# Gotbread/sdf-playground

Measured on AMD Instinct MI355X. Metric: Mrays/s (primary+secondary), labyrinth scene, 3840x2160, higher is better.
Workload: dtype f32

## Files before the change

sdf_playground_amd/buildlib.py:

```python
import hashlib
import os
import re
import subprocess
import sys
from concurrent.futures import ThreadPoolExecutor

HERE = os.path.dirname(os.path.abspath(__file__))
CSRC = os.path.join(HERE, "csrc")
LIB = os.path.join(HERE, "libsdfr.so")
OBJDIR = os.path.join(HERE, "build")
SOURCES = ["sdfr_api.cpp", "sdfr_comm.cpp", "sdfr_hlsl.cpp", "sdfr_jit.cpp", "sdfr_kernels.hip", "sdfr_post.hip"]
GROUP_SOURCE = "sdfr_kernels_group.hip"
ARCH = "gfx950"
_REV = ["-mllvm", "-greedy-reverse-local-assignment"]
_MAXMEM = ["-mllvm", "-amdgpu-sched-strategy=max-memory-clause"]
_TOPDOWN = ["-mllvm", "-misched-prera-direction=topdown"]
_MAXILP = ["-mllvm", "-amdgpu-sched-strategy=max-ilp"]
SCENE_FLAGS = {"SceneFractal": _MAXILP, "SceneCoordinateMaterial": _REV, "SceneTerrain": _REV, "SceneTiling": _REV,
               "SceneCubeSea": _MAXMEM, "SceneShell": _MAXMEM, "SceneLense": _TOPDOWN}


def scene_registry():
    text = open(os.path.join(CSRC, "sdfr_perpixel.h")).read()
    return [(int(i), n) for i, n in re.findall(r"X\((\d+), (Scene\w+)\)", text)]


def group_flags(g, override=None):
    groups = scene_groups()
    flags = []
    table = dict(SCENE_FLAGS)
    table.update(override or {})
    for i, name in scene_registry():
        if i % groups == g:
            flags += [f for f in table.get(name, []) if f not in flags or f == "-mllvm"]
    return flags


FLAGS = ["--offload-arch=" + ARCH, "-std=c++17", "-O3", "-ffp-contract=off", "-fno-slp-vectorize", "-fPIC", "-x", "hip", "-Wno-unused-result",
         "-Wno-unknown-pragmas", "-I" + CSRC]


def scene_groups():
    text = open(os.path.join(CSRC, "sdfr_perpixel.h")).read()
    return int(re.search(r"#define SDFR_GROUPS (\d+)", text).group(1))


def _deps():
    return [os.path.join(CSRC, f) for f in os.listdir(CSRC)] + [os.path.join(os.path.dirname(HERE), "include", "sdfr.h")]


def _stale():
    if not os.path.exists(LIB):
        return True
    t = os.path.getmtime(LIB)
    return any(os.path.getmtime(d) > t for d in _deps())


def build(force=False, verbose=False, extra=(), out=None, jobs=None, scene_flags=None):
    if out is None and not force and not _stale():
        return LIB
    hipcc = os.environ.get("HIPCC", "/opt/rocm/bin/hipcc")
    extra = list(extra)
    objdir = os.path.join(OBJDIR, hashlib.sha1(" ".join(extra).encode()).hexdigest()[:10] if extra else "default")
    os.makedirs(objdir, exist_ok=True)
    units = [(s, [], os.path.join(objdir, s + ".o")) for s in SOURCES]
    for g in range(scene_groups()):
        flags = group_flags(g, scene_flags)
        tag = "" if flags == group_flags(g) else "." + hashlib.sha1(" ".join(flags).encode()).hexdigest()[:8]
        units.append((GROUP_SOURCE, ["-DSDFR_GROUP=%d" % g] + flags, os.path.join(objdir, "%s.%d%s.o" % (GROUP_SOURCE, g, tag))))
    newest_dep = max(os.path.getmtime(d) for d in _deps())

    def compile_unit(u):
        src, defs, obj = u
        if not force and os.path.exists(obj) and os.path.getmtime(obj) > newest_dep:
            return
        cmd = [hipcc] + FLAGS + extra + defs + ["-c", os.path.join(CSRC, src), "-o", obj]
        if verbose:
            print(" ".join(cmd), file=sys.stderr)
        subprocess.run(cmd, check=True)

    with ThreadPoolExecutor(max_workers=jobs or min(8, os.cpu_count() or 1)) as pool:
        list(pool.map(compile_unit, sorted(units, key=lambda u: u[0] != GROUP_SOURCE)))
    cmd = [hipcc, "--offload-arch=" + ARCH, "-fPIC", "-shared"] + [u[2] for u in units] + ["-o", out or LIB]
    if verbose:
        print(" ".join(cmd), file=sys.stderr)
    subprocess.run(cmd, check=True)
    return out or LIB


if __name__ == "__main__":
    build(force="--force" in sys.argv, verbose="-v" in sys.argv)
    print(LIB)
```

sdf_playground_amd/csrc/sdfr_pixel.h:

```cpp
#pragma once
#include "sdfr_frame.h"
#include "sdfr_lib.h"

namespace sdfr {

struct PixelRay
{
	vec3 dir;
	vec3 right_ray, bottom_ray;
};
SDF_HD PixelRay pixel_ray(const FrameU &U, int px, int py)
{
	float sx = ((float)px + 0.5f) / U.widthf * 2.f - 1.f;
	float sy = 1.f - ((float)py + 0.5f) / U.heightf * 2.f;
	vec3 d = U.front + sx * U.right + sy * U.top;
	float invlen = rcp1(length(d));
	PixelRay r;
	r.dir = d * invlen;
	r.right_ray = U.ddx * U.right * invlen;
	r.bottom_ray = U.ddy * U.top * invlen;
	return r;
}
SDF_HD RayRec primary_ray(const FrameU &U, const PixelRay &pr)
{
// ... 11 lines not shown
	f.has_transparent = ray_has_transparent(r);
	f.is_shadow = ray_is_shadow(r);
	f.last_transparent_pos = f.has_transparent ? r.pos : V3s(0.f);
	return f;
}

SDF_HD int queue_next(uint64_t depths, int slots)
{
	int best = 0;
	uint32_t best_depth = (uint32_t)(depths & 0xffu);
	for (int i = 1; i < slots; ++i)
	{
		uint32_t d = (uint32_t)((depths >> (8 * i)) & 0xffu);
		if (d < best_depth) { best = i; best_depth = d; }
	}
	return best;
}
SDF_HD int queue_free(uint64_t depths, int slots)
{
	int i = 0;
	for (; i < slots; ++i)
		if (((depths >> (8 * i)) & 0xffu) == RAY_DEPTH_INVALID) break;
	return i;
}
SDF_HD uint64_t queue_set_depth(uint64_t depths, int slot, uint32_t d)
{
	return (depths & ~(0xffull << (8 * slot))) | ((uint64_t)d << (8 * slot));
}
#define SDFR_QUEUE_EMPTY 0xffffffffffffffffull

struct DebugFlags
{
	int plane_on;
	int show_on;
};
SDF_HD DebugFlags debug_flags(const FrameU &U)
{
	DebugFlags f;
	f.plane_on = U.debug_plane_on;
	f.show_on = U.show_on;
#if defined(__HIP_DEVICE_COMPILE__)
	asm volatile("" : "+v"(f.plane_on), "+v"(f.show_on));
#endif
	return f;
}
SDF_HD bool frame_needs_debug(const FrameU &U) { return U.debug_plane_on != 0 || U.show_on == 0; }

template <class Scene, bool DBG>
SDF_HD float map_geometry(const FrameU &U, const DebugFlags &F, const typename Scene::RayInv &R, vec3 p, vec3 dir, bool fast)
{
	if (!DBG)
		return Scene::dist(U, R, p, dir, fast);
	float d = 3e38f;
	if (F.show_on)
		d = Scene::dist(U, R, p, dir, fast);
	if (F.plane_on)
	{
		float plane = sd_plane_fast(p - V3(U.debug_x, U.debug_y, U.debug_z), dir, fast, U.debug_normal);
		return min1(d, plane);
	}
	return d;
}

struct GeoStep
{
	float camera_distance;
	vec3 right_off, bottom_off;
};
template <bool B>
struct VoidIf {};
template <>
struct VoidIf<true> { typedef void type; };
template <class Scene, class = void>
struct SceneReadsMarchState { static constexpr bool value = false; };
template <class Scene>
struct SceneReadsMarchState<Scene, typename VoidIf<Scene::geometry_reads_march_state>::type> { static constexpr bool value = true; };

template <class Scene, bool DBG>
SDF_HD float map_geometry_at(const FrameU &U, const DebugFlags &F, const typename Scene::RayInv &R, vec3 p, vec3 dir, bool fast, const GeoStep &gs)
{
	if (!DBG)
		return Scene::dist(U, R, p, dir, fast, gs);
	float d = 3e38f;
	if (F.show_on)
		d = Scene::dist(U, R, p, dir, fast, gs);
	if (F.plane_on)
	{
		float plane = sd_plane_fast(p - V3(U.debug_x, U.debug_y, U.debug_z), dir, fast, U.debug_normal);
		return min1(d, plane);
	}
	return d;
}

struct March
{
	vec3 start, dir;
	float t;
	float last_d;
	float last_safe;
	float factor;
	float d;
	uint32_t iter;
};
enum { MARCH_CONTINUE = 0, MARCH_HIT = 1, MARCH_MISS = 2 };

SDF_HD March march_begin(vec3 start, vec3 dir)
{
	March m;
	m.start = start;
	m.dir = dir;
	m.t = 0.f;
	m.last_d = 0.f;
	m.last_safe = 0.f;
	m.factor = 1.f;
	m.d = 0.f;
	m.iter = 0;
	return m;
}
SDF_HD vec3 march_pos(const March &m) { return mad(m.dir, m.t, m.start); }

SDF_HD int march_advance(March &m, float d, float dist_max, uint32_t iter_count, float dist_eps)
{
	m.d = d;
	const bool over = (m.factor > 1.f) & ((m.last_d + d) < m.last_d * m.factor);
	const bool out_of_range = m.t > dist_max;
	const bool stop = !over & (out_of_range | (d < dist_eps));
	const float t_fwd = m.t + d * m.factor;
	const float safe_fwd = m.t + d;
	m.last_d = over ? m.last_d : d;
	m.t = stop ? m.t : (over ? m.last_safe : t_fwd);
	m.last_safe = (over | stop) ? m.last_safe : safe_fwd;
	m.factor = over ? 1.f : m.factor;
	if (stop) return out_of_range ? MARCH_MISS : MARCH_HIT;
	m.iter++;
	return m.iter < iter_count ? MARCH_CONTINUE : MARCH_MISS;
}
SDF_HD void march_pre(March &m) { if (m.iter == 3) m.factor = 1.5f; }

SDF_HD vec3 grad_sample_pos(vec3 p, int axis, float eps)
{
	if (axis == 0) return p + V3(eps, 0.f, 0.f);
	if (axis == 1) return p + V3(0.f, eps, 0.f);
	return p + V3(0.f, 0.f, eps);
}

template <class...>
struct VoidOfN { typedef void type; };
template <class Scene, class = void>
struct SceneNormal
{
	static constexpr bool available = false;
	static SDF_HD void call(const FrameU &, const SurfacePoint &, NormalOut &) {}
};
template <class Scene>
struct SceneNormal<Scene, typename VoidOfN<decltype(&Scene::normal)>::type>
{
	static constexpr bool available = true;
	static SDF_HD void call(const FrameU &U, const SurfacePoint &sp, NormalOut &no) { Scene::normal(U, sp, no); }
};
template <class Scene>
SDF_HD NormalOut scene_normal(const FrameU &U, vec3 hit_pos, vec3 dir, float camera_distance, vec3 right_ray, vec3 bottom_ray)
{
	NormalOut no;
	no.sample_dist = U.grad_eps;
	no.normal = V3s(0.f);
	no.use_normal = false;
	if (SceneNormal<Scene>::available)
	{
		SurfacePoint sp;
		sp.pos = hit_pos;
		sp.dir = dir;
		sp.camera_distance = camera_distance;
		sp.right_off = right_ray;
		sp.bottom_off = bottom_ray;
		sp.normal = V3s(0.f);
		sp.iteration_count = 0u;
		sp.scene_distance = 0.f;
		SceneNormal<Scene>::call(U, sp, no);
	}
	return no;
}

template <class Scene, class = void>
struct SceneLights
{
	static constexpr bool available = false;
	static SDF_HD void call(const FrameU &, const SurfacePoint &, Light *, bool *, float &) {}
};
template <class Scene>
struct SceneLights<Scene, typename VoidOfN<decltype(&Scene::lights)>::type>
{
	static constexpr bool available = true;
	static SDF_HD void call(const FrameU &U, const SurfacePoint &sp, Light *L, bool *used, float &ambient) { Scene::lights(U, sp, L, used, ambient); }
};
template <class Scene, bool HasLights = SceneLights<Scene>::available>
struct SceneAmbient { static SDF_HD float get() { return Scene::ambient(); } };
template <class Scene>
struct SceneAmbient<Scene, true> { static SDF_HD float get() { return 0.075f; } };
template <class Scene, bool HasLights = SceneLights<Scene>::available>
struct SceneLightSlot { static SDF_HD bool get(const FrameU &U, int i, Light &L) { return Scene::light(U, i, L); } };
template <class Scene>
struct SceneLightSlot<Scene, true> { static SDF_HD bool get(const FrameU &, int, Light &) { return false; } };

struct HitInfo
{
	vec3 pos;
	float t;
	float d;
	uint32_t iter;
	vec3 normal;
	float sample_dist;
};

template <class Store>
struct Spawner
{
	Store &store;
	uint64_t depths;
	int count;
	int slots;
	SDF_HD Spawner(Store &s, uint64_t d, int c, int n) : store(s), depths(d), count(c), slots(n) {}
	SDF_HD void push(const RayRec &r)
	{
		if (count < slots)
		{
			int slot = queue_free(depths, slots);
			store.put(slot, r);
			depths = queue_set_depth(depths, slot, ray_depth(r));
			++count;
		}
	}
};

SDF_HD Material default_material(const FrameU &U, vec3 hit_pos)
{
	Material m;
	m.id = MAT_NONE;
	m.mpos = hit_pos;
	m.prop_x = 0.f;
	m.diffuse = V4(0.f, 0.f, 0.f, 1.f);
	m.specular = V4(0.f, 0.f, 0.f, 60.f);
	m.emissive = V3s(0.f);
	m.reflection = V3s(0.f);
	m.refraction = V3s(0.f);
	m.ior = 1.4f;
	m.normal = V4(0.f, 0.f, 0.f, 0.f);
	m.max_cost = U.max_cost_default;
	m.use_hdr = true;
	return m;
}

template <class Scene, bool DBG>
SDF_HD void map_material(const FrameU &U, const DebugFlags &F, const SurfacePoint &sp, Material &m)
{
	if (!DBG)
	{
		Scene::material(U, sp, m);
		return;
	}
	bool on_debug_plane = false;
	if (F.plane_on)
	{
		float plane = sd_plane(sp.pos - V3(U.debug_x, U.debug_y, U.debug_z), U.debug_normal);
		on_debug_plane = on_surface(U, plane);
	}
	if (on_debug_plane)
	{
		RayFlags nf;
		nf.has_transparent = false;
		nf.is_shadow = false;
		nf.last_transparent_pos = V3s(0.f);
		typename Scene::RayInv R0 = Scene::ray_setup(U, sp.dir, nf);
		float d;
		if constexpr (SceneReadsMarchState<Scene>::value)
		{
			GeoStep gs;
			gs.camera_distance = sp.camera_distance;
			gs.right_off = sp.right_off;
			gs.bottom_off = sp.bottom_off;
			d = Scene::dist(U, R0, sp.pos, sp.dir, false, gs);
		}
		else
			d = Scene::dist(U, R0, sp.pos, sp.dir, false);
		m.id = MAT_DISTANCE_PLANE;
		m.prop_x = d / U.debug_scale;
	}
	else
	{
		Scene::material(U, sp, m);
	}
}

template <class Scene, class = void>
struct RayEscapes
{
	static constexpr bool available = false;
	template <class R> static SDF_HD bool test(const FrameU &, const R &, vec3, vec3) { return false; }
};
template <class Scene>
struct RayEscapes<Scene, typename VoidOfN<decltype(&Scene::ray_escapes)>::type>
{
	static constexpr bool available = true;
	template <class R> static SDF_HD bool test(const FrameU &U, const R &r, vec3 p, vec3 dir) { return Scene::ray_escapes(U, r, p, dir); }
};

template <class Scene, class = void>
struct EscapesFrom
{
	static constexpr bool available = false;
	static SDF_HD float get(const FrameU &, vec3, vec3, float) { return 3e38f; }
};
template <class Scene>
struct EscapesFrom<Scene, typename VoidOfN<decltype(&Scene::escapes_from)>::type>
{
	static constexpr bool available = true;
	static SDF_HD float get(const FrameU &U, vec3 start, vec3 dir, float range) { return Scene::escapes_from(U, start, dir, range); }
};
template <class Scene, class = void>
struct InlineEscapedShadows { static constexpr bool value = false; };
template <class Scene>
struct InlineEscapedShadows<Scene, typename VoidOfN<decltype(Scene::inline_escaped_shadows)>::type>
{
	static constexpr bool value = Scene::inline_escaped_shadows && RayEscapes<Scene>::available;
};
struct InlineShadows
{
	vec3 acc;
	int budget;
	int taken;
};

template <class Scene, class Table, class Used>
SDF_HD bool light_in_slot(const FrameU &U, int i, const Table &table, const Used &table_used, Light &L)
{
	bool used = SceneLightSlot<Scene>::get(U, i, L);
	if (SceneLights<Scene>::available)
	{
		L = table[i];
		used = table_used[i];
	}
	if (i >= 1 && i <= U.extension_lights)
	{
		const float *E = U.ext_light[i - 1];
		L.pos = V3(E[0], E[1], E[2]);
		L.directional = false;
		L.extend = 0.25f;
		L.falloff = 0.25f;
		L.color = V3(E[3], E[4], E[5]);
		used = true;
	}
	return used;
}
SDF_HD vec3 light_colour(const Light &L)
{
	float falloff = 1.f;
	if (!L.directional) falloff = pow1(0.1f, L.falloff);
	return L.color * falloff;
}

template <class Scene, bool DBG, class Store, bool INL = false>
SDF_HD vec3 shade_hit(const FrameU &U, const DebugFlags &F, const RayRec &ray, const PixelRay &px, const HitInfo &hit, float max_range,
	float &hdr, Spawner<Store> &q, InlineShadows *inl = nullptr)
{
	bool added = false;
	const uint32_t depth = ray_depth(ray);
	const float inside_sign = ray_inside_sign(ray);
	const vec3 view_dir = ray.dir;

	SurfacePoint sp;
	sp.pos = hit.pos;
	sp.dir = ray.dir;
	sp.camera_distance = hit.t;
	sp.right_off = px.right_ray;
	sp.bottom_off = px.bottom_ray;
	sp.normal = hit.normal;
	sp.iteration_count = hit.iter;
	sp.scene_distance = hit.d;

	Material m = default_material(U, hit.pos);
	map_material<Scene, DBG>(U, F, sp, m);
	if (U.extension_marble_reflection != 0.f && (m.id == MAT_MARBLE_DARK || m.id == MAT_MARBLE_LIGHT)) m.reflection = V3s(U.extension_marble_reflection);

	vec3 out = V3s(0.f);
	if (!ray_is_shadow(ray))
	{
		float new_hdr = m.use_hdr ? 1.f : 0.f;
		hdr = lerp1(hdr, new_hdr, step1(hdr, 0.f));

		vec3 n = lerp(hit.normal, V3(m.normal.x, m.normal.y, m.normal.z), m.normal.w);

		if (any3(m.reflection) && inside_sign > 0.f && depth + 3 < m.max_cost)
		{
			vec3 rv = reflect(view_dir, n);
			RayRec c;
			c.pos = mad(rv, U.reflect_eps, hit.pos);
			c.dir = rv;
			c.contrib = m.reflection * ray.contrib;
			c.shadow_range = 0.f;
			c.bits = depth + 3;
			q.push(c);
		}
		if (any3(m.refraction) && depth + 4 < m.max_cost)
		{
			RayRec c;
			vec3 rv;
			if (inside_sign > 0.f)
			{
				rv = refract(view_dir, n, 1.f / m.ior);
				c.bits = (depth + 2) | RAY_INSIDE;
			}
			else
			{
				rv = refract(view_dir, -n, m.ior);
				c.bits = depth + 2;
			}
			c.pos = mad(rv, U.refract_eps, hit.pos);
			c.dir = rv;
			c.contrib = m.refraction * ray.contrib;
			c.shadow_range = 0.f;
			q.push(c);
		}

		vec3 diffuse = V3(m.diffuse.x, m.diffuse.y, m.diffuse.z);
		vec3 color = V3s(0.f);
		bool use_light = true;
		switch (m.id)
		{
		case MAT_ITER:
			color = color + mat_iter_heat(hit.iter, (uint32_t)(U.iter_count - 1));
			use_light = false;
			hdr = 0.f;
			break;
		case MAT_PLAIN:
			color = color + diffuse;
			use_light = false;
			break;
		case MAT_NORMAL1:
		{
			vec3 nc = max(n, 0.01f);
			nc = nc / max1(max1(nc.x, nc.y), nc.z);
			color = color + nc;
			use_light = false;
			hdr = 0.f;
			break;
		}
		case MAT_NORMAL2:
			color = color + abs(n);
			use_light = false;
			hdr = 0.f;
			break;
		case MAT_DISTANCE_PLANE:
			color = color + mat_debug_plane(m.prop_x);
			use_light = false;
			hdr = 0.f;
			break;
		case MAT_WOOD:
			diffuse = diffuse + mat_wood(m.mpos);
			break;
		case MAT_MARBLE_DARK:
			diffuse = diffuse + mat_marble(m.mpos, V3(0.556f, 0.478f, 0.541f));
			break;
		case MAT_MARBLE_LIGHT:
			diffuse = diffuse + mat_marble(m.mpos, V3(0.7f, 0.7f, 0.7f));
			break;
		case MAT_FIRE:
		{
			float fadeout = sat1(dot(-view_dir, n));
			vec4 fc = mat_fire(m.mpos, 1.f - fadeout);
			color = color + V3(fc.x, fc.y, fc.z);
			m.diffuse = V4(1.f, 1.f, 1.f, sat1(fc.w));
			break;
		}
		default:
			break;
		}

		if (m.diffuse.w < 1.f && depth + 2 < m.max_cost)
		{
			RayRec c;
			c.pos = hit.pos;
			c.dir = view_dir;
			c.contrib = (1.f - m.diffuse.w) * V3(m.diffuse.x, m.diffuse.y, m.diffuse.z) * ray.contrib;
			c.shadow_range = 0.f;
			c.bits = (depth + 2) | RAY_TRANSPARENT;
			q.push(c);
		}

		if (use_light)
		{
			float ambient = SceneAmbient<Scene>::get();
			Light table[SceneLights<Scene>::available ? SDFR_MAX_LIGHTS : 1];
			bool table_used[SceneLights<Scene>::available ? SDFR_MAX_LIGHTS : 1];
			if (SceneLights<Scene>::available)
			{
				for (int i = 0; i < SDFR_MAX_LIGHTS; ++i)
				{
					table_used[i] = false;
					table[i].pos = V3s(0.f);
					table[i].directional = false;
					table[i].extend = 0.f;
					table[i].color = V3s(0.f);
					table[i].falloff = 0.f;
				}
				SceneLights<Scene>::call(U, sp, table, table_used, ambient);
			}
			float move = max1(U.shadow_eps, hit.sample_dist) + max1(0.f, -hit.d);
			vec3 lit_pos = mad(n, move, hit.pos);
			const float alpha = sat1(m.diffuse.w);

			if constexpr (INL)
			{
				for (int i = 0; i < U.light_count; ++i)
				{
					Light L;
					if (!light_in_slot<Scene>(U, i, table, table_used, L)) continue;
					color = color + diffuse * light_colour(L) * ambient;
				}
				color = color + m.emissive;
				color = color * alpha;
				out = out + color * ray.contrib;
				inl->acc = inl->acc + out;
				added = true;
				for (int i = 0; i < U.light_count; ++i)
				{
					Light L;
					if (!light_in_slot<Scene>(U, i, table, table_used, L)) continue;
					vec3 ldir;
					float trace_dist;
					if (L.directional)
					{
						ldir = L.pos / (length(L.pos) + U.dist_eps);
						trace_dist = U.range;
					}
					else
					{
						ldir = lit_pos - L.pos;
						trace_dist = length(ldir);
						ldir = ldir / trace_dist;
						trace_dist = trace_dist - L.extend;
					}
					const vec3 lcol = light_colour(L);
					float ndl = sat1(dot(-n, ldir));
					vec3 direct = V3s(0.f) + diffuse * lcol * ndl;
					vec3 half_vec = -normalize(view_dir + ldir);
					float spec = pow1(sat1(dot(n, half_vec)), m.specular.w);
					direct = direct + V3(m.specular.x, m.specular.y, m.specular.z) * lcol * spec;
					if (depth + 2 < m.max_cost && ndl > 0.f)
					{
						RayRec c;
						c.pos = lit_pos;
						c.dir = -ldir;
						c.contrib = direct * ray.contrib * alpha;
						c.shadow_range = trace_dist;
						c.bits = (depth + 2) | RAY_SHADOW;
						if (inl->taken + q.count >= q.slots) continue;
						if (U.step_shortcuts != 0 && q.count == 0 && inl->taken < inl->budget)
						{
							const typename Scene::RayInv R = Scene::ray_setup(U, c.dir, ray_flags(c));
							March sm = march_begin(c.pos, c.dir);
							march_pre(sm);
							if (sm.factor == 1.f && RayEscapes<Scene>::test(U, R, march_pos(sm), c.dir))
							{
								inl->acc = inl->acc + (V3s(0.f) + c.contrib);
								inl->taken++;
								q.store.ray_marched(c, 0u, MARCH_MISS);
								continue;
							}
						}
						q.push(c);
					}
				}
			}
			else
			for (int i = 0; i < U.light_count; ++i)
			{
				Light L;
				bool used = SceneLightSlot<Scene>::get(U, i, L);
				if (SceneLights<Scene>::available)
				{
					L = table[i];
					used = table_used[i];
				}
				if (i >= 1 && i <= U.extension_lights)
				{
					const float *E = U.ext_light[i - 1];
					L.pos = V3(E[0], E[1], E[2]);
					L.directional = false;
					L.extend = 0.25f;
					L.falloff = 0.25f;
					L.color = V3(E[3], E[4], E[5]);
					used = true;
				}
				if (!used) continue;
				vec3 ldir;
				float trace_dist;
				float falloff = 1.f;
				if (L.directional)
				{
					ldir = L.pos / (length(L.pos) + U.dist_eps);
					trace_dist = U.range;
				}
				else
				{
					ldir = lit_pos - L.pos;
					trace_dist = length(ldir);
					ldir = ldir / trace_dist;
// ... 60 lines not shown
```

sdf_playground_amd/csrc/sdfr_render_pixel.h:

```cpp
#pragma once
#include "sdfr_pixel.h"

namespace sdfr {


struct LocalRayStore
{
	RayRec slot[SDFR_MAX_RAYS];
	SDF_HD void put(int i, const RayRec &r) { slot[i] = r; }
	SDF_HD RayRec get(int i) const { return slot[i]; }
	SDF_HD void ray_marched(const RayRec &, uint32_t, int) {}
};

template <class Backing>
struct CachedRayStore
{
	Backing &backing;
	RayRec cached;
	int cached_slot;
	PixelRay kept;
	float hdr;
	SDF_HD explicit CachedRayStore(Backing &b) : backing(b), cached_slot(-1) {}
	SDF_HD void keep_pixel_ray(const PixelRay &pr) { kept = pr; }
	SDF_HD PixelRay pixel_ray_kept() const { return kept; }
	SDF_HD void keep_hdr(float h) { hdr = h; }
	SDF_HD float hdr_kept() const { return hdr; }
	SDF_HD void ray_marched(const RayRec &r, uint32_t iter, int status) { backing.ray_marched(r, iter, status); }
	SDF_HD void put(int i, const RayRec &r)
	{
		if (cached_slot >= 0) backing.put(cached_slot, cached);
		cached = r;
		cached_slot = i;
	}
	SDF_HD RayRec get(int i)
	{
		if (i == cached_slot)
		{
			cached_slot = -1;
			return cached;
		}
		return backing.get(i);
	}
};

template <class...>
struct VoidOf { typedef void type; };
template <class Scene, class = void>
struct ShadowHitsNeedNormal { static constexpr bool value = true; };
template <class Scene>
struct ShadowHitsNeedNormal<Scene, typename VoidOf<decltype(Scene::shadow_hits_need_normal)>::type>
{
	static constexpr bool value = Scene::shadow_hits_need_normal;
};

template <class Scene, class = void>
struct PersistentTiles { static constexpr bool value = false; };
template <class Scene>
struct PersistentTiles<Scene, typename VoidOf<decltype(Scene::persistent_tiles)>::type>
{
	static constexpr bool value = Scene::persistent_tiles;
};

template <class Scene, class = void>
struct SquareUnits { static constexpr bool value = false; };
template <class Scene>
struct SquareUnits<Scene, typename VoidOf<decltype(Scene::square_units)>::type> { static constexpr bool value = Scene::square_units; };

template <class Scene, class = void>
struct SceneTileShape { static constexpr int value = 3; };
template <class Scene>
struct SceneTileShape<Scene, typename VoidOf<decltype(Scene::tile_w_log2)>::type> { static constexpr int value = Scene::tile_w_log2; };

template <class Scene, class = void>
struct RetireAfter { static constexpr int value = 8; };
template <class Scene>
struct RetireAfter<Scene, typename VoidOf<decltype(Scene::retire_after)>::type> { static constexpr int value = Scene::retire_after; };

struct PixelCounters
{
	uint32_t rays, march_evals, hits;
#ifdef SDFR_PHASE_CLOCKS
	uint64_t clk_march, clk_grad, clk_shade, clk_miss, clk_total;
#endif
};
#ifdef SDFR_PHASE_CLOCKS
#define SDFR_CLK(var) const uint64_t var = __builtin_readcyclecounter()
#define SDFR_CLK_ADD(field, t0, t1) cnt.field += (t1) - (t0)
#else
#define SDFR_CLK(var)
#define SDFR_CLK_ADD(field, t0, t1)
#endif

template <class Scene, bool DBG, class Store>
SDF_HD vec4 render_pixel(const FrameU &U, int px, int py, PixelCounters &cnt, Store &store)
{
	SDFR_CLK(c_begin);
	constexpr bool INL = !DBG && InlineEscapedShadows<Scene>::value;
	const DebugFlags F = debug_flags(U);
	RayRec ray;
	{
		const PixelRay pr = pixel_ray(U, px, py);
		ray = primary_ray(U, pr);
		store.keep_pixel_ray(pr);
	}
	uint64_t depths = SDFR_QUEUE_EMPTY;
	int count = 0;

	store.keep_hdr(-1.f);
	vec3 acc = V3s(0.f);
	for (int bounce = 0; bounce < U.bounce_count; ++bounce)
	{
		if (bounce > 0)
		{
			if (count == 0) break;
			const int idx = queue_next(depths, U.ray_count);
			ray = store.get(idx);
			depths = queue_set_depth(depths, idx, RAY_DEPTH_INVALID);
			--count;
		}
		cnt.rays++;

		const typename Scene::RayInv R = Scene::ray_setup(U, ray.dir, ray_flags(ray));
		const float inside_sign = ray_inside_sign(ray);
		const float max_range = ray_is_shadow(ray) ? ray.shadow_range : U.range;

		SDFR_CLK(c0);
		March m = march_begin(ray.pos, ray.dir);
		int status;
		const uint32_t evals_before = cnt.march_evals;
		const bool shortcuts = !DBG && (RayEscapes<Scene>::available || EscapesFrom<Scene>::available) && U.step_shortcuts != 0 && inside_sign > 0.f;
		float clear_from = 3e38f;
		if constexpr (EscapesFrom<Scene>::available)
			if (shortcuts) clear_from = EscapesFrom<Scene>::get(U, ray.pos, ray.dir, max_range);
		do
		{
			march_pre(m);
			bool escaped = shortcuts && RayEscapes<Scene>::test(U, R, march_pos(m), ray.dir);
			if constexpr (EscapesFrom<Scene>::available) escaped = escaped || m.t >= clear_from;
			if (escaped && m.factor == 1.f)
			{
				status = MARCH_MISS;
				break;
			}
			float d;
			if constexpr (SceneReadsMarchState<Scene>::value)
			{
				const PixelRay pr = store.pixel_ray_kept();
				GeoStep gs;
				gs.camera_distance = m.t;
				gs.right_off = pr.right_ray;
				gs.bottom_off = pr.bottom_ray;
				d = map_geometry_at<Scene, DBG>(U, F, R, march_pos(m), ray.dir, true, gs) * inside_sign;
			}
			else
				d = map_geometry<Scene, DBG>(U, F, R, march_pos(m), ray.dir, true) * inside_sign;
			cnt.march_evals++;
			if (escaped && !((m.last_d + d) < m.last_d * m.factor))
			{
				status = MARCH_MISS;
				break;
			}
			status = march_advance(m, d, max_range, (uint32_t)U.iter_count, U.dist_eps);
		} while (status == MARCH_CONTINUE);
		SDFR_CLK(c1);
		SDFR_CLK_ADD(clk_march, c0, c1);
		store.ray_marched(ray, cnt.march_evals - evals_before, status);

		vec3 out;
		if (status == MARCH_HIT)
		{
			cnt.hits++;
			HitInfo hit;
			hit.pos = march_pos(m);
			hit.t = m.t;
			hit.d = m.d;
			hit.iter = m.iter;
			hit.normal = V3s(0.f);
			hit.sample_dist = U.grad_eps;
			if (ShadowHitsNeedNormal<Scene>::value || !ray_is_shadow(ray))
			{
				NormalOut no;
				if (SceneNormal<Scene>::available)
				{
					const PixelRay pr = store.pixel_ray_kept();
					no = scene_normal<Scene>(U, hit.pos, ray.dir, hit.t, pr.right_ray, pr.bottom_ray);
				}
				else
					no = scene_normal<Scene>(U, hit.pos, ray.dir, hit.t, V3s(0.f), V3s(0.f));
				hit.sample_dist = no.sample_dist;
				hit.normal = no.normal;
				if (!no.use_normal)
				{
					const float baseline = m.d * inside_sign;
					float g0, g1, g2;
					if constexpr (SceneReadsMarchState<Scene>::value)
					{
						const PixelRay pr = store.pixel_ray_kept();
						GeoStep gs;
						gs.camera_distance = hit.t;
						gs.right_off = pr.right_ray;
						gs.bottom_off = pr.bottom_ray;
						g0 = map_geometry_at<Scene, DBG>(U, F, R, grad_sample_pos(hit.pos, 0, no.sample_dist), ray.dir, false, gs) - baseline;
						g1 = map_geometry_at<Scene, DBG>(U, F, R, grad_sample_pos(hit.pos, 1, no.sample_dist), ray.dir, false, gs) - baseline;
						g2 = map_geometry_at<Scene, DBG>(U, F, R, grad_sample_pos(hit.pos, 2, no.sample_dist), ray.dir, false, gs) - baseline;
					}
					else
					{
						g0 = map_geometry<Scene, DBG>(U, F, R, grad_sample_pos(hit.pos, 0, no.sample_dist), ray.dir, false) - baseline;
						g1 = map_geometry<Scene, DBG>(U, F, R, grad_sample_pos(hit.pos, 1, no.sample_dist), ray.dir, false) - baseline;
						g2 = map_geometry<Scene, DBG>(U, F, R, grad_sample_pos(hit.pos, 2, no.sample_dist), ray.dir, false) - baseline;
					}
					hit.normal = normalize(V3(g0, g1, g2));
				}
			}
#ifdef SDFR_PHASE_CLOCKS
			asm volatile("" : "+v"(hit.normal.x), "+v"(hit.normal.y), "+v"(hit.normal.z));
#endif
			SDFR_CLK(c2);
			SDFR_CLK_ADD(clk_grad, c1, c2);

			Spawner<Store> q(store, depths, count, U.ray_count);
			float hdr = store.hdr_kept();
			if constexpr (INL)
			{
				InlineShadows inl;
				inl.acc = acc;
				inl.budget = U.bounce_count - 1 - bounce;
				inl.taken = 0;
				out = shade_hit<Scene, DBG, Store, true>(U, F, ray, store.pixel_ray_kept(), hit, max_range, hdr, q, &inl);
				acc = inl.acc;
				bounce += inl.taken;
				cnt.rays += (uint32_t)inl.taken;
			}
			else
				out = shade_hit<Scene, DBG, Store>(U, F, ray, store.pixel_ray_kept(), hit, max_range, hdr, q);
			store.keep_hdr(hdr);
			depths = q.depths;
			count = q.count;
#ifdef SDFR_PHASE_CLOCKS
			asm volatile("" : "+v"(out.x), "+v"(out.y), "+v"(out.z));
#endif
			SDFR_CLK(c3);
			SDFR_CLK_ADD(clk_shade, c2, c3);
			if constexpr (!INL) acc = acc + out;
		}
		else
		{
			out = shade_miss<Scene>(U, ray, m.iter);
#ifdef SDFR_PHASE_CLOCKS
			asm volatile("" : "+v"(out.x), "+v"(out.y), "+v"(out.z));
#endif
			SDFR_CLK(c4);
			SDFR_CLK_ADD(clk_miss, c1, c4);
			acc = acc + out;
		}
	}
	SDFR_CLK(c_end);
	SDFR_CLK_ADD(clk_total, c_begin, c_end);
	return V4(acc.x, acc.y, acc.z, abs1(store.hdr_kept()));
}

}
```

sdf_playground_amd/csrc/sdfr_scenes.h:

```cpp
#pragma once
#include "sdfr_frame.h"
#include "sdfr_lib.h"

namespace sdfr {

struct SceneFastSphere
{
	static const char *name() { return "fast_sphere"; }
	static constexpr bool shadow_hits_need_normal = false;
	static const char *variables() { return ""; }
	static SDF_HD void prepare(FrameU &) {}
	struct RayInv { GroundInv ground; };
	static SDF_HD RayInv ray_setup(const FrameU &U, vec3 dir, const RayFlags &)
	{
		RayInv r;
		r.ground = ground_setup(dir);
		return r;
	}
	static SDF_HD bool ray_escapes(const FrameU &U, const RayInv &, vec3 p, vec3 dir) { return ray_leaves_floor_and_ball(p, dir, 1.51f, V3(0.f, 1.f, 0.f), 0.52f); }
	static constexpr bool inline_escaped_shadows = true;
	static SDF_HD float dist(const FrameU &U, const RayInv &R, vec3 p, vec3 dir, bool fast)
	{
		float d = min1(3e38f, ground_dist(p, fast, R.ground));
		return min1(d, sd_sphere_fast(p - V3(0.f, 1.f, 0.f), dir, fast, 0.5f, U.dist_eps));
	}
	static SDF_HD void material(const FrameU &U, const SurfacePoint &sp, Material &m)
	{
		ground_material(U, sp, m);
		if (on_surface(U, sd_sphere(sp.pos - V3(0.f, 1.f, 0.f), 0.5f)))
		{
			m.diffuse = V4(0.2f, 0.7f, 0.2f, 1.f);
			set_rgb(m.specular, 0.5f);
		}
	}
	static SDF_HD bool light(const FrameU &U, int i, Light &L) { return sun_light(i, L); }
	static SDF_HD float ambient() { return 0.075f; }
	static SDF_HD vec3 background(const FrameU &U, vec3 dir, uint32_t) { return sky_color(dir, U.sky_s, U.sky_c); }
};

struct SceneCubeSea
{
	static const char *name() { return "cube_sea"; }
	static constexpr bool persistent_tiles = true;
	static constexpr int retire_after = 4;
	static constexpr bool shadow_hits_need_normal = false;
	static const char *variables() { return ""; }
	static SDF_HD void prepare(FrameU &) {}
	struct RayInv { GroundInv ground; vec2 barrier; vec2 rdir; bool exact_x, exact_z, rising; };
	static SDF_HD RayInv ray_setup(const FrameU &U, vec3 dir, const RayFlags &)
	{
		RayInv r;
		r.ground = ground_setup(dir);
		r.barrier = (V2(step1(0.f, dir.x), step1(0.f, dir.z)) - 0.5f) * V2(2.01f, 2.01f);
		r.exact_x = abs1(dir.x) >= 8.6736174e-19f;
		r.exact_z = abs1(dir.z) >= 8.6736174e-19f;
		r.rdir = V2(r.exact_x ? rcp1(dir.x) : 0.f, r.exact_z ? rcp1(dir.z) : 0.f);
		r.rising = dir.y >= 0.f;
		return r;
	}
	static SDF_HD bool ray_escapes(const FrameU &U, const RayInv &R, vec3 p, vec3) { return R.rising && p.y > 3.66f; }
	static SDF_HD float guard_quotient(float num, float den, float rden, bool exact)
	{
		if (exact) return div_c(num, den, rden);
		return num / den;
	}
	struct Cell { vec3 cell_pos; float cube; bool is_other; };
	static SDF_HD vec3 cell_position(vec3 p)
	{
		vec2 rep = op_rep_inf(V2(p.x, p.z), V2(2.f, 2.f));
		return V3(rep.x, p.y, rep.y);
	}
	static SDF_HD Cell eval_cell(const FrameU &U, vec3 p)
	{
		Cell c;
		c.cell_pos = cell_position(p);
		const vec2 rep = V2(c.cell_pos.x, c.cell_pos.z);
		vec2 cell_index = (V2(p.x, p.z) - rep) / 2.f;
		vec2 q = cell_index * 0.5f + 0.25f;
		vec2 sometimes = V2(rne1(frac1(q.x)), rne1(frac1(q.y)));
		c.is_other = sometimes.x < 0.5f && sometimes.y < 0.5f;
		float phase = cell_index.x + cell_index.y * 0.3f + U.stime;
		vec2 sc = sincos1(phase);
		vec2 rsc = sincos1_small(sc.y * 0.4f);
		vec2 r = rot2(rep, rsc.x, rsc.y);
		vec3 cube_pos = V3(r.x, p.y, r.y);
		float hs = c.is_other ? 0.25f : 0.5f;
		c.cube = sd_box(cube_pos - V3(0.f, 2.f + sc.x, 0.f), V3s(hs)) - 0.15f;
		return c;
	}
	static SDF_HD float cube_lower_bound(vec3 p, bool *valid)
	{
		*valid = p.y < 1024.f;
		return max1(p.y - 3.66f, 0.34f - p.y);
	}
	static SDF_HD float dist(const FrameU &U, const RayInv &R, vec3 p, vec3 dir, bool fast)
	{
		const vec3 cell_pos = cell_position(p);
		const vec2 num = R.barrier - V2(cell_pos.x, cell_pos.z);
		const float tx = guard_quotient(num.x, dir.x, R.rdir.x, R.exact_x);
		const float tz = guard_quotient(num.y, dir.z, R.rdir.y, R.exact_z);
		const float d = min1(min1(3e38f, ground_dist(p, fast, R.ground)), min1(tx, tz));
		bool valid;
		const float lb = cube_lower_bound(p, &valid);
		if (valid && lb >= d) return d;
		return min1(d, eval_cell(U, p).cube);
	}
	static SDF_HD void material(const FrameU &U, const SurfacePoint &sp, Material &m)
	{
		ground_material(U, sp, m);
		Cell c = eval_cell(U, sp.pos);
		if (on_surface(U, c.cube))
		{
			if (c.is_other)
			{
				m.diffuse = V4(0.8f, 0.2f, 0.2f, 1.f);
				set_rgb(m.specular, 1.f);
			}
			else
			{
				m.diffuse = V4(0.6f, 0.5f, 0.2f, 1.f);
				set_rgb(m.specular, 1.f);
				m.reflection = V3s(0.25f);
			}
		}
	}
	static SDF_HD bool light(const FrameU &U, int i, Light &L) { return sun_light(i, L); }
	static SDF_HD float ambient() { return 0.075f; }
	static SDF_HD vec3 background(const FrameU &U, vec3 dir, uint32_t) { return sky_color(dir, U.sky_s, U.sky_c); }
};

struct SceneLabyrinth
{
	static const char *name() { return "labyrinth"; }
	static constexpr int waves_per_simd = 7;
	static constexpr bool persistent_tiles = true;
	static constexpr int retire_after = 4;
	static constexpr bool shadow_hits_need_normal = false;
	static const char *variables() { return ""; }
	enum { SU_FIRE_SCROLL = 0 };
	static SDF_HD void prepare(FrameU &U) { U.su[SU_FIRE_SCROLL] = U.stime * 3.f; }

	static SDF_HD float fire_cone(vec3 p) { return sd_round_cone(p, V3(0.f, 1.1f, 0.f), V3(0.f, 1.6f, 0.f), 0.15f, 0.1f); }

	struct RayInv { GroundInv ground; bool skip_fire, rising; };
	static SDF_HD RayInv ray_setup(const FrameU &U, vec3 dir, const RayFlags &f)
	{
		RayInv r;
		r.ground = ground_setup(dir);
		r.skip_fire = f.has_transparent && fire_cone(f.last_transparent_pos) < U.dist_eps;
		r.rising = dir.y >= 0.f;
		return r;
	}
	static SDF_HD bool ray_escapes(const FrameU &U, const RayInv &R, vec3 p, vec3) { return R.rising && p.y > 4.01f; }

	static SDF_HD float vase(vec3 p)
	{
		float bowl = sd_sphere(p - V3(0.f, 1.89f, 0.f), 0.5f);
		float stem = sd_capped_cylinder(p - V3(0.f, 0.8f, 0.f), 0.75f, 0.2f);
		float foot = sd_box(p - V3(0.f, 0.075f, 0.f), V3(0.4f, 0.075f, 0.4f));
		float cut_top = sd_plane(p - V3(0.f, 1.9f, 0.f), V3(0.f, 1.f, 0.f));
		float cut_low = sd_plane(p - V3(0.f, 1.5f, 0.f), V3(0.f, -1.f, 0.f));
		float d = max1(bowl, cut_low);
		d = op_pipe_merge_c(d, stem, 0.1f, 4.f);
		d = op_pipe_merge_c(d, foot, 0.1f, 4.f);
		d = max1(d, cut_top);
		d = max1(d, -bowl - 0.06f);
		return d;
	}

	static SDF_HD vec3 fold(vec3 p)
	{
		vec2 rep = op_rep_inf_c(V2(p.x, p.z), 20.f, 1.0f / 20.f);
		float wx = abs1(rep.x), wz = abs1(rep.y);
		if (wz > wx) { float t = wx; wx = wz; wz = t; }
		return V3(wx, p.y, wz);
	}
	static SDF_HD float walls(vec3 wp)
	{
		float wall1 = sd_box(wp - V3(3.5f, 2.f, 3.f), V3(1.5f, 2.f, 1.f));
		float wall2 = sd_box(wp - V3(7.f, 2.f, 5.f), V3(3.f, 2.f, 1.f));
		return min1(wall1, wall2);
	}
	static SDF_HD vec3 vase_local(vec3 wp) { return V3(abs1(wp.x - 8.f), wp.y, wp.z) - V3(1.f, 0.f, 3.f); }
	struct Torch { float wood, fire; vec3 torch_pos; };
	static SDF_HD Torch torch(vec3 wp)
	{
		Torch t;
		const float torch_angle = 15.f * SDFR_PI / 180.f;
		const float tc = cos1(torch_angle), ts = sin1(torch_angle);
		vec3 tp = wp - V3(5.f, 2.f, 3.f);
		vec3 sp = V3(tp.x * tc - tp.y * ts, tp.x * ts + tp.y * tc, tp.z);
		tp.x = tp.x - 0.3f;
		t.wood = sd_box(sp - V3(0.f, 0.6f, 0.f), V3(0.05f, 0.5f, 0.05f));
		t.fire = fire_cone(tp);
		t.torch_pos = tp;
		return t;
	}

	static SDF_HD bool beyond(vec3 v, float reach, float radius)
	{
		const float k = reach + radius;
		return dot(v, v) >= k * k;
	}
	static SDF_HD float dist(const FrameU &U, const RayInv &R, vec3 p, vec3, bool fast)
	{
		float d = min1(3e38f, ground_dist(p, fast, R.ground));
		const vec3 wp = fold(p);
		d = min1(d, walls(wp));
		if (max1(max1(4.28f - wp.x, wp.y - 3.82f), abs1(wp.z - 3.f) - 1.52f) >= max1(d, 0.f)) return d;
		const vec3 q = vase_local(wp);
		if (!beyond(q - V3(0.f, 1.2f, 0.f), max1(d, 0.f), 1.35f + 0.15f + 0.01f))
			d = min1(d, vase(q));
		if (!beyond(wp - V3(5.f, 2.f, 3.f) - V3(0.2f, 0.9f, 0.f), max1(d, 0.f), 0.9f + 0.01f))
		{
			const Torch t = torch(wp);
			d = min1(d, t.wood);
			d = R.skip_fire ? d : min1(d, t.fire);
		}
		return d;
	}
	static SDF_HD void material(const FrameU &U, const SurfacePoint &sp, Material &m)
	{
		ground_material(U, sp, m);
		const vec3 wp = fold(sp.pos);
		if (on_surface(U, walls(wp)))
		{
			m.mpos = sp.pos;
			m.id = MAT_MARBLE_LIGHT;
			return;
		}
		const vec3 q = vase_local(wp);
		if (!beyond(q - V3(0.f, 1.2f, 0.f), U.dist_eps, 1.35f + 0.15f + 0.01f) && on_surface(U, vase(q)))
		{
			m.mpos = sp.pos * 3.f;
			m.id = MAT_MARBLE_DARK;
			return;
		}
		if (beyond(wp - V3(5.f, 2.f, 3.f) - V3(0.2f, 0.9f, 0.f), U.dist_eps, 0.9f + 0.01f)) return;
		const Torch t = torch(wp);
		if (on_surface(U, t.wood))
		{
			m.mpos = V3(sp.pos.x, sp.pos.z, sp.pos.y) * 2.f;
			m.id = MAT_WOOD;
		}
		else if (on_surface(U, t.fire))
		{
			m.mpos = t.torch_pos * 3.f - V3(0.f, U.su[SU_FIRE_SCROLL], 0.f);
			m.id = MAT_FIRE;
		}
	}
	static SDF_HD bool light(const FrameU &U, int i, Light &L) { return sun_light(i, L); }
	static SDF_HD float ambient() { return 0.075f; }
	static SDF_HD vec3 background(const FrameU &U, vec3 dir, uint32_t) { return sky_color(dir, U.sky_s, U.sky_c); }
};

struct SceneFractal
{
	static const char *name() { return "fractal"; }
	static constexpr bool square_units = true;
	static constexpr int retire_after = 1;
	static constexpr int waves_per_simd = 7;
	static constexpr bool persistent_tiles = true;
	static constexpr bool shadow_hits_need_normal = false;
	static const char *variables() { return ""; }
	static SDF_HD void prepare(FrameU &) {}
	struct RayInv { GroundInv ground; bool rising; };
	static SDF_HD RayInv ray_setup(const FrameU &U, vec3 dir, const RayFlags &)
	{
		RayInv r;
		r.ground = ground_setup(dir);
		r.rising = dir.y >= 0.f;
		return r;
	}
	static SDF_HD bool ray_escapes(const FrameU &U, const RayInv &, vec3 p, vec3 dir) { return ray_leaves_floor_and_ball(p, dir, 2.01f, V3(0.f, 1.f, 0.f), 1.02f); }
	static constexpr bool inline_escaped_shadows = true;
	static SDF_HD float fold(vec3 p, float *level_hit)
	{
		const float size = 1.f;
		vec3 q = p - V3(0.f, 1.f, 0.f);
		float d = 1e30f;
		float scale = 1.f;
		float hit_level = 0.f;
#pragma unroll
		for (int i = 0; i < 8; ++i)
		{
			float nd = div_c(sd_box(q, V3s(size * 0.5f)), scale, 1.0f / scale);
			if (nd < 0.0001f && d > 0.0001f) hit_level = (float)i;
			d = min1(d, nd);
			q = abs(q);
			sort3_desc(q.y, q.x, q.z);
			q.y = q.y - size * 2.f / 3.f;
			q.y = q.y + size / 3.f;
			sort3_desc(q.y, q.x, q.z);
			q.y = q.y - size / 3.f;
			q = q * 3.f;
			scale = scale * 3.f;
		}
		*level_hit = hit_level;
		return d;
	}
	static SDF_HD float fold_below(vec3 p, float d)
	{
		const float size = 1.f;
		vec3 q = p - V3(0.f, 1.f, 0.f);
		float scale = 1.f;
#pragma unroll
		for (int i = 0; i < 8; ++i)
		{
			const float k = max1(d, 0.f) * scale + (1.f + 0.01f);
			if (dot(q, q) >= k * k) return d;
			d = min1(d, div_c(sd_box(q, V3s(size * 0.5f)), scale, 1.0f / scale));
			q = abs(q);
			sort3_desc(q.y, q.x, q.z);
			q.y = q.y - size * 2.f / 3.f;
			q.y = q.y + size / 3.f;
			sort3_desc(q.y, q.x, q.z);
			q.y = q.y - size / 3.f;
			q = q * 3.f;
			scale = scale * 3.f;
		}
		return d;
	}
	static SDF_HD float dist(const FrameU &U, const RayInv &R, vec3 p, vec3, bool fast)
	{
		return fold_below(p, min1(3e38f, ground_dist(p, fast, R.ground)));
	}
	static SDF_HD void material(const FrameU &U, const SurfacePoint &sp, Material &m)
	{
		ground_material(U, sp, m);
		float lvl;
		float d = fold(sp.pos, &lvl);
		if (on_surface(U, d))
		{
			m.diffuse.x = 0.9f;
			m.diffuse.y = 0.7f;
			m.diffuse.z = lvl * 0.125f;
			set_rgb(m.specular, 0.5f);
		}
	}
	static SDF_HD bool light(const FrameU &U, int i, Light &L) { return sun_light(i, L); }
	static SDF_HD float ambient() { return 0.075f; }
	static SDF_HD vec3 background(const FrameU &U, vec3 dir, uint32_t) { return sky_color(dir, U.sky_s, U.sky_c); }
};

struct SceneLense
{
	static const char *name() { return "lense"; }
	static constexpr int tile_w_log2 = 4;
	static constexpr int waves_per_simd = 8;
	static constexpr bool persistent_tiles = true;
	static constexpr bool shadow_hits_need_normal = false;
	static const char *variables()
	{
		return "VAR_xpos(min = -4, max = 4, step = 0.1) VAR_ypos(min = -4, max = 4, step = 0.1) "
			   "VAR_zpos(min = 0, max = 25, step = 0.1) VAR_mixing(min = 0, max = 1, step = 0.05)";
	}
	enum { SV_XPOS = 0, SV_YPOS = 1, SV_ZPOS = 2, SV_MIXING = 3 };
	enum { SU_MIRROR_S = 0, SU_MIRROR_C = 1 };
	static SDF_HD void prepare(FrameU &U)
	{
		vec2 sc = sincos1(U.stime * 0.3f);
		U.su[SU_MIRROR_S] = sc.x;
		U.su[SU_MIRROR_C] = sc.y;
	}
	struct RayInv { int unused; };
	static SDF_HD RayInv ray_setup(const FrameU &U, vec3, const RayFlags &) { RayInv r; r.unused = 0; return r; }

	struct Objects { float bg1, bg2, lense, sphere, mirror, frame; vec3 mirror_pos; vec2 bg1_xz; };
	static SDF_HD float blob(vec3 p)
	{
		return lerp1(sd_sphere(p, 1.f), sd_box(p, V3s(1.f)), 0.65f) - 0.1f;
	}
	static SDF_HD Objects eval_objects(const FrameU &U, vec3 p)
	{
		Objects o;
		vec3 b1 = p - V3(0.f, -5.f, 0.f);
		vec2 r1 = op_rep_inf_c(V2(b1.x, b1.z), 3.f, 1.0f / 3.f);
		o.bg1_xz = r1;
		o.bg1 = blob(V3(r1.x, b1.y, r1.y));

		vec3 b2 = p - V3(0.f, 5.f, 0.f);
		vec2 r2 = op_rep_inf_c(V2(b2.x, b2.z), 10.f, 1.0f / 10.f);
		o.bg2 = blob(V3(r2.x, b2.y, r2.y));

		vec3 lp = abs(p);
		lp.z = lp.z - 5.1f;
		o.lense = max1(-sd_sphere(lp, 5.f), sd_sphere(p, 2.f));

		o.sphere = sd_sphere(p - V3(U.scene_var[SV_XPOS], U.scene_var[SV_YPOS], U.scene_var[SV_ZPOS]), 2.f);

		vec3 mp = p - V3(0.f, 0.f, -5.f);
		vec2 mr = rot2(V2(mp.x, mp.z), U.su[SU_MIRROR_S], U.su[SU_MIRROR_C]);
		mp = V3(mr.x, mp.y, mr.y);
		o.mirror_pos = mp;
		o.mirror = sd_box(mp, V3(1.f, 2.f, 0.1f));
		o.frame = sd_box(mp, V3(1.1f, 2.1f, 0.08f));
		return o;
	}
	static SDF_HD float blob_field_lower_bound(float h) { return abs1(h) - 1.11f; }
	static SDF_HD bool ball_is_farther(vec3 p, vec3 c, float radius, float d)
	{
		const vec3 v = p - c;
		const float k = max1(d, 0.f) + (radius + 0.01f);
		return dot(v, v) >= k * k;
	}
	static SDF_HD float ball_left_behind(vec3 start, vec3 dir, vec3 c, float radius)
	{
		const vec3 v = start - c;
		const float b = dot(v, dir), cc = dot(v, v) - radius * radius, dd = dot(dir, dir);
		const float disc = b * b - cc * dd;
		if (disc < 0.f) return 0.f;
		return (sqrt1(disc) - b) / dd + 0.01f;
	}
	static SDF_HD float escapes_from(const FrameU &U, vec3 start, vec3 dir, float range)
	{
		const float y_end = start.y + dir.y * range;
		float t = 0.f;
		if (!(abs1(y_end) < 3.86f))
		{
			if (!(dir.y > 1e-3f) || !(y_end > 6.2f)) return 3e38f;
			const float inv = 1.f / dir.y;
			const float ta = (max1(start.y, 3.86f) - start.y) * inv, tb = max1((6.14f - start.y) * inv, 0.f);
			const float xa = start.x + dir.x * ta, xb = start.x + dir.x * tb, za = start.z + dir.z * ta, zb = start.z + dir.z * tb;
			const float xl = (min1(xa, xb) - 1.13f) * 0.1f, xh = (max1(xa, xb) + 1.13f) * 0.1f, zl = (min1(za, zb) - 1.13f) * 0.1f, zh = (max1(za, zb) + 1.13f) * 0.1f;
			const bool clear_x = floor1(xl) == floor1(xh) && xl > floor1(xl), clear_z = floor1(zl) == floor1(zh) && zl > floor1(zl);
			if (!((clear_x || clear_z) && abs1(start.x) < 1e4f && abs1(start.z) < 1e4f)) return 3e38f;
			if (start.y < -3.86f) t = (-3.86f - start.y) * inv;
		}
		else if (!(abs1(start.y) < 3.86f)) t = ((start.y > 0.f ? 3.86f : -3.86f) - start.y) / dir.y;
		const vec3 ball = V3(U.scene_var[SV_XPOS], U.scene_var[SV_YPOS], U.scene_var[SV_ZPOS]);
		const float t0 = ball_left_behind(start, dir, V3(0.f, 0.f, 0.f), 2.02f), t1 = ball_left_behind(start, dir, ball, 2.02f), t2 = ball_left_behind(start, dir, V3(0.f, 0.f, -5.f), 2.40f);
		t = max1(max1(t, t0), max1(t1, t2));
		return (t == t && t0 == t0 && t1 == t1 && t2 == t2) ? t : 3e38f;
	}
	static SDF_HD float dist(const FrameU &U, const RayInv &, vec3 p, vec3, bool)
	{
		const bool far_out = !(abs1(p.y) < 1024.f);
		float d = 3e38f;
		const bool near_a_field = abs1(p.y) > 2.9f && !far_out;
		if (near_a_field)
		{
			vec3 b1 = p - V3(0.f, -5.f, 0.f);
			if (!(blob_field_lower_bound(b1.y) >= d))
			{
				vec2 r1 = op_rep_inf_c(V2(b1.x, b1.z), 3.f, 1.0f / 3.f);
				d = min1(d, blob(V3(r1.x, b1.y, r1.y)));
			}
			vec3 b2 = p - V3(0.f, 5.f, 0.f);
			if (!(blob_field_lower_bound(b2.y) >= d))
			{
				vec2 r2 = op_rep_inf_c(V2(b2.x, b2.z), 10.f, 1.0f / 10.f);
				d = min1(d, blob(V3(r2.x, b2.y, r2.y)));
			}
		}
		if (!near_a_field || !ball_is_farther(p, V3(0.f, 0.f, 0.f), 2.f, d))
		{
// ... 247 lines not shown
```

Measured before the change: 11110.

## Compute per-ray clear height in labyrinth to escape rising rays earlier

Adds a start-position-aware ray_setup for the labyrinth scene. For each rising ray it traces the folded, mirrored cell geometry (wall boxes and balls) analytically to find the height above which the ray cannot hit anything, and uses that height as the escape threshold instead of the fixed 4.01. This is meant to end marching of secondary and sky-bound rays sooner. It adds a loop of up to 16 iterations of setup arithmetic per ray, plus register pressure, and its correctness depends on the analytic bounds matching the SDF. The labyrinth scene also gets the reverse-local-assignment register allocator flag.

```diff
diff --git a/sdf_playground_amd/buildlib.py b/sdf_playground_amd/buildlib.py
--- a/sdf_playground_amd/buildlib.py
+++ b/sdf_playground_amd/buildlib.py
@@ -16,7 +16,7 @@
 _MAXMEM = ["-mllvm", "-amdgpu-sched-strategy=max-memory-clause"]
 _TOPDOWN = ["-mllvm", "-misched-prera-direction=topdown"]
 _MAXILP = ["-mllvm", "-amdgpu-sched-strategy=max-ilp"]
-SCENE_FLAGS = {"SceneFractal": _MAXILP, "SceneCoordinateMaterial": _REV, "SceneTerrain": _REV, "SceneTiling": _REV,
+SCENE_FLAGS = {"SceneFractal": _MAXILP, "SceneCoordinateMaterial": _REV, "SceneTerrain": _REV, "SceneTiling": _REV, "SceneLabyrinth": _REV,
                "SceneCubeSea": _MAXMEM, "SceneShell": _MAXMEM, "SceneLense": _TOPDOWN}
 
 
diff --git a/sdf_playground_amd/csrc/sdfr_pixel.h b/sdf_playground_amd/csrc/sdfr_pixel.h
--- a/sdf_playground_amd/csrc/sdfr_pixel.h
+++ b/sdf_playground_amd/csrc/sdfr_pixel.h
@@ -337,6 +337,18 @@
 {
 	static constexpr bool available = true;
 	template <class R> static SDF_HD bool test(const FrameU &U, const R &r, vec3 p, vec3 dir) { return Scene::ray_escapes(U, r, p, dir); }
+};
+template <class Scene, class = void>
+struct RaySetupAtStart
+{
+	static constexpr bool available = false;
+	static SDF_HD typename Scene::RayInv call(const FrameU &U, vec3, vec3 dir, const RayFlags &f) { return Scene::ray_setup(U, dir, f); }
+};
+template <class Scene>
+struct RaySetupAtStart<Scene, typename VoidOfN<decltype(Scene::ray_setup(*(const FrameU *)0, *(const vec3 *)0, *(const vec3 *)0, *(const RayFlags *)0))>::type>
+{
+	static constexpr bool available = true;
+	static SDF_HD typename Scene::RayInv call(const FrameU &U, vec3 start, vec3 dir, const RayFlags &f) { return Scene::ray_setup(U, start, dir, f); }
 };
 
 template <class Scene, class = void>
diff --git a/sdf_playground_amd/csrc/sdfr_render_pixel.h b/sdf_playground_amd/csrc/sdfr_render_pixel.h
--- a/sdf_playground_amd/csrc/sdfr_render_pixel.h
+++ b/sdf_playground_amd/csrc/sdfr_render_pixel.h
@@ -120,7 +120,7 @@
 		}
 		cnt.rays++;
 
-		const typename Scene::RayInv R = Scene::ray_setup(U, ray.dir, ray_flags(ray));
+		const typename Scene::RayInv R = RaySetupAtStart<Scene>::call(U, ray.pos, ray.dir, ray_flags(ray));
 		const float inside_sign = ray_inside_sign(ray);
 		const float max_range = ray_is_shadow(ray) ? ray.shadow_range : U.range;
 
diff --git a/sdf_playground_amd/csrc/sdfr_scenes.h b/sdf_playground_amd/csrc/sdfr_scenes.h
--- a/sdf_playground_amd/csrc/sdfr_scenes.h
+++ b/sdf_playground_amd/csrc/sdfr_scenes.h
@@ -142,16 +142,90 @@
 
 	static SDF_HD float fire_cone(vec3 p) { return sd_round_cone(p, V3(0.f, 1.1f, 0.f), V3(0.f, 1.6f, 0.f), 0.15f, 0.1f); }
 
-	struct RayInv { GroundInv ground; bool skip_fire, rising; };
+	struct RayInv { GroundInv ground; float clear_y; bool skip_fire, rising; };
 	static SDF_HD RayInv ray_setup(const FrameU &U, vec3 dir, const RayFlags &f)
 	{
 		RayInv r;
 		r.ground = ground_setup(dir);
 		r.skip_fire = f.has_transparent && fire_cone(f.last_transparent_pos) < U.dist_eps;
 		r.rising = dir.y >= 0.f;
+		r.clear_y = 4.01f;
 		return r;
 	}
-	static SDF_HD bool ray_escapes(const FrameU &U, const RayInv &R, vec3 p, vec3) { return R.rising && p.y > 4.01f; }
+	static SDF_HD RayInv ray_setup(const FrameU &U, vec3 start, vec3 dir, const RayFlags &f)
+	{
+		RayInv r = ray_setup(U, dir, f);
+		if (r.rising) r.clear_y = clear_height(start, dir, min1(4.f + 2.f * U.dist_eps + 1e-5f, 4.01f));
+		return r;
+	}
+	static SDF_HD bool ray_escapes(const FrameU &U, const RayInv &R, vec3 p, vec3) { return R.rising && p.y > R.clear_y; }
+
+	static SDF_HD void clip_slab(float x, float u, float ru, float lo, float hi, float &t0, float &t1)
+	{
+		if (u == 0.f)
+		{
+			if (!(x >= lo && x <= hi)) t1 = -1.f;
+			return;
+		}
+		const float a = (lo - x) * ru, b = (hi - x) * ru;
+		t0 = max1(t0, min1(a, b));
+		t1 = min1(t1, max1(a, b));
+	}
+	static SDF_HD float rect_exit(vec2 p, vec2 u, vec2 ru, float tmax, float x0, float x1, float z0, float z1)
+	{
+		float t0 = 0.f, t1 = tmax;
+		clip_slab(p.x, u.x, ru.x, x0, x1, t0, t1);
+		clip_slab(p.y, u.y, ru.y, z0, z1, t0, t1);
+		return t0 <= t1 ? t1 : -1.f;
+	}
+	static SDF_HD float ball_exit(vec2 p, float y, vec2 u, float dy, float uu, float ruu, float tmax, vec3 c, float radius)
+	{
+		const float vx = p.x - c.x, vy = y - c.y, vz = p.y - c.z;
+		const float b = vx * u.x + vy * dy + vz * u.y;
+		const float disc = b * b - uu * (vx * vx + vy * vy + vz * vz - radius * radius);
+		if (!(disc >= 0.f)) return -1.f;
+		const float q = sqrt1(disc);
+		const float t0 = (-b - q) * ruu, t1 = (q - b) * ruu;
+		return t1 >= 0.f && t0 <= tmax ? min1(t1, tmax) : -1.f;
+	}
+	static SDF_HD float clear_height(vec3 s, vec3 dir, float top)
+	{
+		const float h = sqrt1(dir.x * dir.x + dir.z * dir.z);
+		const float ry = rcp1(dir.y);
+		const float t_top = (top - s.y) * ry;
+		if (!(s.y < top) || !(dir.y > 0.01f * h) || !(t_top * h <= 20.f)) return top;
+		const float uu = dir.x * dir.x + dir.y * dir.y + dir.z * dir.z, ruu = rcp1(uu);
+		vec2 p = op_rep_inf_c(V2(s.x, s.z), 20.f, 1.0f / 20.f), u = V2(dir.x, dir.z);
+		if (p.x < 0.f) { p.x = -p.x; u.x = -u.x; }
+		if (p.y < 0.f) { p.y = -p.y; u.y = -u.y; }
+		if (p.y > p.x) { p = V2(p.y, p.x); u = V2(u.y, u.x); }
+		vec2 ru = V2(rcp1(u.x), rcp1(u.y));
+		float t = 0.f, blocked = -1.f;
+		for (int k = 0; k < 16; ++k)
+		{
+			float te = t_top - t;
+			int edge = 0;
+			if (u.y < 0.f && -p.y * ru.y < te) { te = -p.y * ru.y; edge = 1; }
+			if (u.y > u.x && (p.x - p.y) * rcp1(u.y - u.x) < te) { te = (p.x - p.y) * rcp1(u.y - u.x); edge = 2; }
+			if (u.x > 0.f && (10.f - p.x) * ru.x < te) { te = (10.f - p.x) * ru.x; edge = 3; }
+			te = max1(te, 0.f);
+			const float e1 = rect_exit(p, u, ru, te, 1.99f, 5.01f, 1.99f, 4.01f);
+			const float e2 = rect_exit(p, u, ru, te, 3.99f, 10.01f, 3.99f, 6.01f);
+			const float y = fma1(dir.y, t, s.y);
+			const float e3 = ball_exit(p, y, u, dir.y, uu, ruu, te, V3(7.f, 1.2f, 3.f), 1.52f);
+			const float e4 = ball_exit(p, y, u, dir.y, uu, ruu, te, V3(9.f, 1.2f, 3.f), 1.52f);
+			const float e5 = ball_exit(p, y, u, dir.y, uu, ruu, te, V3(5.2f, 2.9f, 3.f), 0.92f);
+			const float e = max1(max1(max1(e1, e2), e3), max1(e4, e5));
+			if (e >= 0.f) blocked = t + e;
+			if (edge == 0) return blocked < 0.f ? 1e-20f : min1(max1(fma1(dir.y, blocked, s.y), 1e-20f), top);
+			p = V2(fma1(u.x, te, p.x), fma1(u.y, te, p.y));
+			t += te;
+			if (edge == 1) { p.y = 0.f; u.y = -u.y; ru.y = -ru.y; }
+			else if (edge == 2) { p.x = p.y = 0.5f * (p.x + p.y); u = V2(u.y, u.x); ru = V2(ru.y, ru.x); }
+			else { p.x = 10.f; u.x = -u.x; ru.x = -ru.x; }
+		}
+		return top;
+	}
 
 	static SDF_HD float vase(vec3 p)
 	{
```

Measured after the change: 11220, median of 6. Within noise of the previous version (+1.0%).
